# JacobYoung115/VisualSLAM

Measured on AMD Instinct MI355X. Metric: frames/sec @1080p (Harris + DoG keypoint detection), higher is better.
Workload: dtype u8

## Files before the change

### visualslam_amd/csrc/kernels_hdiff.hip.h

```cpp
#pragma once
#include <hip/hip_runtime.h>

#include <utility>
#include <vector>

#include "diff_taps.gen.h"
#include "kernels_strip.hip.h"
#include "vslam_internal.h"

namespace vslam {

typedef float hd_f2 __attribute__((ext_vector_type(2)));

template <class F, int... I>
__device__ __forceinline__ void hd_for_impl(F&& f, std::integer_sequence<int, I...>) {
    (f(std::integral_constant<int, I>{}), ...);
}
template <int N, class F>
__device__ __forceinline__ void hd_for(F&& f) {
    hd_for_impl(f, std::make_integer_sequence<int, N>{});
}

__host__ __device__ constexpr int hd_phys(int c) { return c + (c >> 4) * HD_PAD; }

template <class LV>
__host__ __device__ constexpr int hd_w(int k) { return k >= 0 && k < LV::n ? (int)LV::w[k] : 0; }

template <class LV>
__host__ __device__ constexpr int hd_coef(int e) {
    if (LV::form == 1) {
        for (int i = 0; i < LV::nd; ++i)
            if (LV::de[i] == e) return LV::dc[i];
        return 0;
    }
    return hd_w<LV>(e + LV::n / 2);
}

template <int O>
struct HdGeom {
    static constexpr int nmax = dtaps::Lvl<O, 5>::n;
    static constexpr int rmax = nmax / 2;
    static constexpr int HL = hd_left_halo(rmax);
    static_assert(dtaps::Lvl<O, 0>::n <= nmax && dtaps::Lvl<O, 4>::n <= nmax, "level 5 is the widest");
};

template <class LV, int HL>
__device__ __forceinline__ void hd_level(const hd_f2* __restrict__ lane, hd_f2 (&acc)[HD_J]) {
    constexpr int n = LV::n, r = n / 2;
    constexpr bool DIFF = LV::form == 1;
    constexpr int lo = DIFF ? -r - 1 : -r, hi = HD_J - 1 + r;
    constexpr int t0 = (HL + lo) & ~1, Q = (HL + hi - t0) / 2 + 1;
    hd_f2 seed = {0.f, 0.f};
    hd_for<HD_J>([&](auto j) { acc[decltype(j)::value] = hd_f2{0.f, 0.f}; });
    hd_for<Q>([&](auto q) {
        constexpr int t = t0 + 2 * decltype(q)::value;
        const float4 v = *reinterpret_cast<const float4*>(lane + hd_phys(t));
        const hd_f2 hv[2] = {hd_f2{v.x, v.y}, hd_f2{v.z, v.w}};
        hd_for<2>([&](auto b) {
            constexpr int x = t + decltype(b)::value - HL;
            if constexpr (DIFF) {
                constexpr int wk = hd_w<LV>(x + 1 + r);
                if constexpr (wk != 0) seed = __builtin_elementwise_fma(hd_f2((float)wk), hv[decltype(b)::value], seed);
            }
            hd_for<HD_J>([&](auto j) {
                constexpr int c = hd_coef<LV>(x - decltype(j)::value);
                if constexpr (c != 0)
                    acc[decltype(j)::value] = __builtin_elementwise_fma(hd_f2((float)c), hv[decltype(b)::value], acc[decltype(j)::value]);
            });
        });
    });
    if constexpr (DIFF) {
        acc[0] += seed;
        hd_for<HD_J - 1>([&](auto j) { acc[decltype(j)::value + 1] += acc[decltype(j)::value]; });
    }
}

template <int O>
__global__ __launch_bounds__(256) void k_gauss_h_diff(const uint16_t* __restrict__ h, size_t hframe, uint8_t* __restrict__ oct_out,
                                                       size_t pframe, int rows, int cols, int pitch, int npairs, int pw,
                                                       uint8_t* __restrict__ next_base, size_t nframe, int nrows, int ncols, int npitch) {
    using G = HdGeom<O>;
    extern __shared__ __attribute__((aligned(16))) uint32_t smem[];
    hd_f2* hp = reinterpret_cast<hd_f2*>(smem);
    const int tid = threadIdx.x;
    const int y0 = blockIdx.y * 2 * npairs;
    const size_t P = (size_t)rows * pitch;
    uint8_t* out = oct_out + blockIdx.z * pframe;
    const int ncs = (cols + HD_J - 1) / HD_J;
    const int ccount = G::HL + HD_J * ncs + G::rmax;
    const int n8 = cols >> 3, nb = ccount - 8 * n8;
    const bool active = tid < npairs * ncs;
    const int ip = tid / ncs, is = tid - ip * ncs;
    const hd_f2* lane = hp + ip * pw + is * (HD_J + HD_PAD);
    const int n8d = max(n8, 1);
    const int i_p0 = tid / n8d, i_k0 = tid - i_p0 * n8d, i_dp = 256 / n8d, i_dk = 256 - i_dp * n8d;
    const int b_p0 = tid / nb, b_i0 = tid - b_p0 * nb, b_dp = 256 / nb, b_di = 256 - b_dp * nb;
    uint32_t prev_e[2][4], prev_o[2][4];

    hd_for<VSLAM_NUM_LEVELS>([&](auto lc) {
        constexpr int L = decltype(lc)::value;
        const uint16_t* hl = h + blockIdx.z * hframe + (size_t)L * P;
        __syncthreads();
        for (int it = tid, p = i_p0, k = i_k0; it < npairs * n8; it += 256, p += i_dp, k += i_dk) {
            if (k >= n8) k -= n8, ++p;
            const uint4 a = *reinterpret_cast<const uint4*>(hl + (size_t)min(y0 + 2 * p, rows - 1) * pitch + 8 * k);
            const uint4 b = *reinterpret_cast<const uint4*>(hl + (size_t)min(y0 + 2 * p + 1, rows - 1) * pitch + 8 * k);
            float4* q = reinterpret_cast<float4*>(hp + p * pw + hd_phys(G::HL + 8 * k));
            const uint32_t av[4] = {a.x, a.y, a.z, a.w}, bv[4] = {b.x, b.y, b.z, b.w};
#pragma unroll
            for (int i = 0; i < 4; ++i)
                q[i] = make_float4((float)(av[i] & 0xffffu), (float)(bv[i] & 0xffffu), (float)(av[i] >> 16), (float)(bv[i] >> 16));
        }
        for (int it = tid, p = b_p0, i = b_i0; it < npairs * nb; it += 256, p += b_dp, i += b_di) {
            if (i >= nb) i -= nb, ++p;
            const int c = i < G::HL ? i : 8 * n8 + i;
            const int x = reflect101(c - G::HL, cols);
            const uint16_t* ra = hl + (size_t)min(y0 + 2 * p, rows - 1) * pitch;
            const uint16_t* rb = hl + (size_t)min(y0 + 2 * p + 1, rows - 1) * pitch;
            hp[p * pw + hd_phys(c)] = hd_f2{(float)ra[x], (float)rb[x]};
        }
        __syncthreads();
        if (active) {
            hd_f2 acc[HD_J];
            hd_level<dtaps::Lvl<O, L>, G::HL>(lane, acc);
            const int x = HD_J * is;
            hd_for<2>([&](auto rc) {
                constexpr int rho = decltype(rc)::value;
                const int y = y0 + 2 * ip + rho;
                uint32_t u[HD_J], g[4], d[4];
                hd_for<HD_J>([&](auto j) { u[decltype(j)::value] = (uint32_t)acc[decltype(j)::value][rho]; });
#pragma unroll
                for (int hw = 0; hw < 4; ++hw) {
                    const uint32_t e = __builtin_amdgcn_perm(u[4 * hw + 2], u[4 * hw + 0], 0x0c060c02);
                    const uint32_t o = __builtin_amdgcn_perm(u[4 * hw + 3], u[4 * hw + 1], 0x0c060c02);
                    g[hw] = __builtin_amdgcn_perm(o, e, 0x06020400);
                    if constexpr (L > 0)
                        d[hw] = __builtin_amdgcn_perm(pk_sub_sat_u16(o, prev_o[rho][hw]), pk_sub_sat_u16(e, prev_e[rho][hw]), 0x06020400);
                    prev_e[rho][hw] = e;
                    prev_o[rho][hw] = o;
                }
                if (y < rows) {
                    const size_t off = (size_t)y * pitch + x;
                    *reinterpret_cast<uint4*>(out + (size_t)L * P + off) = make_uint4(g[0], g[1], g[2], g[3]);
                    if constexpr (L > 0)
                        *reinterpret_cast<uint4*>(out + (size_t)(VSLAM_NUM_LEVELS + L - 1) * P + off) = make_uint4(d[0], d[1], d[2], d[3]);
                    if constexpr (L == 3 && rho == 0)
                        if (next_base && (y >> 1) < nrows && (x >> 1) < ncols)
                            *reinterpret_cast<uint2*>(next_base + blockIdx.z * nframe + (size_t)(y >> 1) * npitch + (x >> 1)) =
                                make_uint2(even_bytes(g[0], g[1]), even_bytes(g[2], g[3]));
                }
            });
        }
    });
}

template <int O, int L>
static bool hd_level_matches(const std::vector<uint16_t>& t) {
    using LV = dtaps::Lvl<O, L>;
    if ((int)t.size() != LV::n) return false;
    for (int k = 0; k < LV::n; ++k)
        if (t[k] != LV::w[k]) return false;
    std::vector<int> off, coef;
    if (diff_form(t.data(), LV::n, off, coef) != LV::form) return false;
    if (LV::form == 1) {
        if ((int)off.size() != LV::nd) return false;
        for (int i = 0; i < LV::nd; ++i)
            if (off[i] != LV::de[i] || coef[i] != LV::dc[i]) return false;
    }
    return true;
}
template <int O>
static bool hd_octave_matches(const std::vector<uint16_t> (&taps)[6]) {
    return hd_level_matches<O, 0>(taps[0]) && hd_level_matches<O, 1>(taps[1]) && hd_level_matches<O, 2>(taps[2]) &&
           hd_level_matches<O, 3>(taps[3]) && hd_level_matches<O, 4>(taps[4]) && hd_level_matches<O, 5>(taps[5]);
}

}
```

### visualslam_amd/csrc/vslam_hip.hip

```cpp
#include <hip/hip_runtime.h>

#include <algorithm>
#include <cstdio>
#include <cstdlib>
#include <cstring>
#include <deque>
#include <map>
#include <string>
#include <set>
#include <memory>
#include <vector>

#include "../../include/vslam.h"
#include "kernels_generic.hip.h"
#include "kernels_pyramid.hip.h"
#include "kernels_strip.hip.h"
#include "kernels_hdiff.hip.h"
#include "kernels_aux.hip.h"
#include "kernels_harris_strip.hip.h"
#include "kernels_orient.hip.h"
#include "kernels_orient_batch.hip.h"
#include "kernels_orient_pk.hip.h"
#include "kernels_compact.hip.h"
#include "kernels_sift.hip.h"
#include "kernels_extrema_dense.hip.h"
#include "vslam_batch_plan.h"
#include "vslam_internal.h"
#include "vslam_ctx.h"
#include "vslam_launch.h"
#include "vslam_mx.h"
#include "vslam_octave_launch.h"

using namespace vslam;


struct vslam_pyramid {
    vslam_ctx* ctx = nullptr;
    vslam_params params{};
    vslam_batch_layout layout{};
    vslam_pyramid_info info{};
    uint8_t* d_block = nullptr;
    uint8_t* d_bases = nullptr;
    size_t block_cap = 0, bases_cap = 0;
    size_t base_off[VSLAM_MAX_OCTAVES] = {};
};


static const char* const kKernelNames =
    "k_resize_linear2x\nk_blur_h_generic\nk_blur_v_generic\n"
    "k_dog5\nk_resize_nearest_half\nk_extrema\nk_pyr_octave\nk_pyr_octave_mx\n"
    "k_gauss_v_strip\nk_gauss_h_strip\nk_gauss_h_diff\nk_resize_linear2x_slide\nk_resize_nearest_half_v4\nk_extrema_w3\nk_extrema_dense\nk_localize_points\nk_orient_keypoints\nk_edge_response_windows\nk_level_gradients\nk_pack_rows\nk_edge_flags\nk_survivor_ranges\nk_orient_survivors\n"
    "k_extrema_pack\nk_harris_strip\nk_flag_count\nk_chunk_scan\nk_flag_scatter\nk_level_gradients\nk_sift_descriptors\nk_pack_offsets\nk_pack_copy\nk_count_totals\n"
    "k_desc_norms\nk_match_nn2\nk_match_merge\n"
    "k_guided_rows\nk_match_guided\nk_match_guided_merge\n"
    "k_guided_hf_rows\nk_guided_hf_kinds\nk_match_guided_hf\n"
    "k_match_nn2_mutual\nk_match_mutual_merge\nk_match_rnn_write\n"
    "k_epi_coords\nk_epi_models\nk_epi_score\nk_epi_select\nk_epi_flags\n"
    "k_refit_init\nk_refit_count\nk_refit_begin\nk_refit_dist\nk_refit_scale\nk_refit_moments\nk_refit_solve\n"
    "k_hom_models\nk_hom_score\nk_hom_select\nk_hom_flags\nk_hom_verdict\n"
    "k_pose_candidates\nk_pose_vote\nk_pose_select\nk_pose_points\n"
    "k_chain_link\nk_chain_ratio\nk_chain_median\nk_chain_walk\nk_chain_map\n"
    "k_res_corr\nk_res_gather\nk_res_models\nk_res_score\nk_res_select\nk_res_flags\n"
    "k_rr_init\nk_rr_pass\nk_rr_step\nk_rr_flags_zero\nk_rr_flags\n"
    "k_trk_next\nk_trk_walk\nk_trk_rows\n"
    "k_ba_init\nk_ba_points\nk_ba_cam_pass\nk_ba_cam_step\nk_ba_member_bits\nk_ba_points_final";


struct StreamSwap {
    vslam_ctx* c;
    hipStream_t saved;
    StreamSwap(vslam_ctx* ctx, hipStream_t s) : c(ctx), saved(ctx->stream) { c->stream = s; }
    ~StreamSwap() { c->stream = saved; }
};

static int raise_dyn_lds(vslam_ctx* c, const void* fn) {
    if (c->lds_raised.count(fn)) return VSLAM_OK;
    HIPCHK(c, hipFuncSetAttribute(fn, hipFuncAttributeMaxDynamicSharedMemorySize, kMaxDynLds));
    c->lds_raised.insert(fn);
    return VSLAM_OK;
}

static void* block_alloc(vslam_ctx* c, size_t bytes, size_t* cap) {
    int best = -1;
    for (int i = 0; i < (int)c->block_cache.size(); ++i) {
        const size_t sz = c->block_cache[i].first;
        if (sz >= bytes && sz <= 2 * bytes + (1 << 20) && (best < 0 || sz < c->block_cache[best].first)) best = i;
    }
    if (best >= 0) {
        void* p = c->block_cache[best].second;
        *cap = c->block_cache[best].first;
        c->block_cache.erase(c->block_cache.begin() + best);
        return p;
    }
    void* p = nullptr;
    if (hipMalloc(&p, bytes) != hipSuccess) {
        for (auto& b : c->block_cache) (void)hipFree(b.second);
        c->block_cache.clear();
        if (hipMalloc(&p, bytes) != hipSuccess) return nullptr;
    }
    *cap = bytes;
    return p;
}
static void block_release(vslam_ctx* c, void* p, size_t cap) {
    if (!p) return;
    if (c && c->block_cache.size() < 8 && cap <= ((size_t)1 << 30))
        c->block_cache.emplace_back(cap, p);
    else
        (void)hipFree(p);
}

int vslam::ws_reserve(vslam_ctx* c, size_t bytes) {
    if (bytes <= c->ws_cap) return VSLAM_OK;
    HIPCHK(c, hipStreamSynchronize(c->stream));
    for (int i = 0; i < vslam_ctx::kAux; ++i)
        if (c->aux[i]) HIPCHK(c, hipStreamSynchronize(c->aux[i]));
    if (c->ws) (void)hipFree(c->ws);
    c->ws = nullptr;
    c->ws_cap = 0;
    const size_t want = align_up(bytes + bytes / 8, 1 << 20);
    HIPCHK(c, hipMalloc((void**)&c->ws, want));
    c->ws_cap = want;
    return VSLAM_OK;
}

static bool stream_is_capturing(vslam_ctx* c) {
    hipStreamCaptureStatus cap = hipStreamCaptureStatusNone;
    if (hipStreamIsCapturing(c->stream, &cap) != hipSuccess) (void)hipGetLastError();
    return cap != hipStreamCaptureStatusNone;
}
#define NO_TABLE_IN_CAPTURE(ctx, what)                                                                                                      \
    if (stream_is_capturing(ctx))                                                                                                           \
    return fail(ctx, VSLAM_ERR_UNSUPPORTED, std::string(what) + ": its tap tables are not on the device yet and cannot be put there during a stream capture - " \
                                                                "run one warm-up call with the same parameters and the same matrix-path setting first")

enum TableKind { kTableBlur, kTableStrip, kTableTile, kTableMx, kTableOrient };

template <class T, class Fill>
static int get_table(vslam_ctx* c, TableKind kind, double v, int i, const char* what, size_t bytes, Fill fill, const T** out) {
    uint64_t vb;
    std::memcpy(&vb, &v, 8);
    const auto key = std::make_tuple((int)kind, vb, i);
    auto it = c->tables.find(key);
    if (it == c->tables.end()) {
        NO_TABLE_IN_CAPTURE(c, what);
        std::vector<char> host(bytes);
        TRY(fill(static_cast<void*>(host.data())));
        void* d = nullptr;
        HIPCHK(c, hipMalloc(&d, bytes));
        HIPCHK(c, hipMemcpy(d, host.data(), bytes, hipMemcpyHostToDevice));
        it = c->tables.emplace(key, d).first;
    }
    *out = static_cast<const T*>(it->second);
    return VSLAM_OK;
}

static inline void tap_pointers(const std::vector<uint16_t> taps[6], const uint16_t* tp[6]) {
    for (int l = 0; l < 6; ++l) tp[l] = taps[l].data();
}

static int get_taps(vslam_ctx* c, int n, double sigma, const uint16_t** out, int* n_eff) {
    std::vector<uint16_t> h;
    if (!gauss_taps_q8_trimmed(n, sigma, h)) return fail(c, VSLAM_ERR_INVALID, "invalid Gaussian kernel size");
    *n_eff = (int)h.size();
    return get_table(c, kTableBlur, sigma, n, "Gaussian blur", sizeof(uint16_t) * h.size(), [&](void* host) -> int {
        std::memcpy(host, h.data(), sizeof(uint16_t) * h.size());
        return VSLAM_OK;
    }, out);
}

static inline dim3 grid_rows(int cols, int rows, int frames = 1) { return dim3((cols + 255) / 256, rows, frames); }


namespace {
enum class OctPath { Tile0, Tile1, Strip, Generic };

struct OctPlan {
    OctPath path = OctPath::Generic;
    int ks[6] = {};
    double sg[6] = {};
    int ke[6] = {};
    std::vector<uint16_t> taps[6];
    int nmax = 0;
    int sh = 0;
    int hdiff = 0;
    int mx = 0;
};
}

static bool taps_fit_u8(const OctPlan& pl) {
    for (int l = 0; l < 6; ++l)
        for (uint16_t v : pl.taps[l])
            if (v > 255) return false;
    return true;
}

template <class CFG>
static bool matches_cfg(const int ks[6]) {
    for (int l = 0; l < 6; ++l)
        if (ks[l] != CFG::n(l)) return false;
    return true;
}

static OctPlan plan_octave(double sigma0, int o, int rows, int cols) {
    OctPlan pl;
    int& nmax = pl.nmax;
    for (int l = 0; l < 6; ++l) {
        pl.sg[l] = sigma_at(sigma0, o, l);
        pl.ks[l] = gauss_ksize_u8(pl.sg[l]);
        if (!gauss_taps_q8_trimmed(pl.ks[l], pl.sg[l], pl.taps[l])) return pl;
        pl.ke[l] = (int)pl.taps[l].size();
        nmax = std::max(nmax, pl.ke[l]);
    }
    if (!taps_fit_u8(pl)) return pl;
    if (matches_cfg<PyrCfgOct0>(pl.ke)) {
        pl.path = OctPath::Tile0;
    } else if (matches_cfg<PyrCfgOct1>(pl.ke)) {
        pl.path = OctPath::Tile1;
    } else if (nmax <= STRIP_MAXN) {
        pl.sh = strip_plan_sh(rows, cols, nmax);
        if (pl.sh) pl.path = OctPath::Strip;
        if (pl.path == OctPath::Strip && hdiff_fits(cols))
            pl.hdiff = hd_octave_matches<2>(pl.taps) ? 2 : hd_octave_matches<3>(pl.taps) ? 3 : 0;
    }
    if (pl.path != OctPath::Generic) pl.mx = mx_config_for(pl.ke);
    return pl;
}

static std::vector<OctPlan> plan_octaves(double sigma0, const vslam_batch_layout& L) {
    std::vector<OctPlan> plans;
    for (int o = 0; o < L.n_octaves; ++o) plans.push_back(plan_octave(sigma0, o, L.rows[o], L.cols[o]));
    return plans;
}

template <int SH, int RI>
static int launch_h_strip(vslam_ctx* c, const uint16_t* h, size_t hframe, const OctIO& io, const StripLaunch& sl, const StripTaps* taps) {
    TRY(raise_dyn_lds(c, reinterpret_cast<const void*>(&k_gauss_h_strip<SH, RI>)));
    LAUNCH_ON(c, "k_gauss_h_strip", c->launch_tag, c->stream, sl.h_lds, (k_gauss_h_strip<SH, RI>), dim3(1, sl.h_grid_y, io.nf), dim3(256), h,
              hframe, io.oct, io.pframe, io.rows, io.cols, io.pitch, sl.pw, taps, io.next_base, io.nframe, io.nrows, io.ncols, io.npitch);
    return VSLAM_OK;
}

template <int O>
static int launch_h_diff(vslam_ctx* c, const uint16_t* h, size_t hframe, const OctIO& io, const StripLaunch& sl) {
    TRY(raise_dyn_lds(c, reinterpret_cast<const void*>(&k_gauss_h_diff<O>)));
    TimedScope ts(c, "k_gauss_h_strip", c->launch_tag);
    LAUNCH_ON(c, "k_gauss_h_diff", c->launch_tag, c->stream, sl.h_lds, k_gauss_h_diff<O>, dim3(1, sl.h_grid_y, io.nf), dim3(256), h,
              hframe, io.oct, io.pframe, io.rows, io.cols, io.pitch, sl.npairs, sl.pw, io.next_base, io.nframe, io.nrows, io.ncols, io.npitch);
    return VSLAM_OK;
}

static int enqueue_strip_octave(vslam_ctx* c, double sigma0, int o, const OctPlan& pl, const OctIO& io, uint16_t* h) {
    const StripTaps* taps;
    TRY(get_table(c, kTableStrip, sigma0, o, "strip kernels", sizeof(StripTaps), [&](void* host) -> int {
        const uint16_t* tp[6];
        tap_pointers(pl.taps, tp);
        if (!strip_pack_taps(tp, pl.ke, *static_cast<StripTaps*>(host))) return fail(c, VSLAM_ERR_UNSUPPORTED, "strip kernels: taps out of range");
        return VSLAM_OK;
    }, &taps));
    const int rows = io.rows, cols = io.cols, nf = io.nf;
    static const bool hdiff_off = [] {
        const char* e = VSLAM_DIAG_ENV("VSLAM_HDIFF");
        return e && e[0] == '0';
    }();
    const int hd = hdiff_off ? 0 : pl.hdiff;
    const StripLaunch sl = hd == 2   ? strip_launch(rows, cols, nf, pl.sh, true, pl.nmax, HdGeom<2>::HL, HdGeom<2>::rmax)
                           : hd == 3 ? strip_launch(rows, cols, nf, pl.sh, true, pl.nmax, HdGeom<3>::HL, HdGeom<3>::rmax)
                                     : strip_launch(rows, cols, nf, pl.sh, false, pl.nmax);
    const StripVGeom vg = strip_v_geom(rows, pl.nmax);
    const size_t P = (size_t)rows * io.pitch;
    TRY(raise_dyn_lds(c, reinterpret_cast<const void*>(&k_gauss_v_strip)));
    LAUNCH_ON(c, "k_gauss_v_strip", o, c->stream, sl.v_lds, k_gauss_v_strip, dim3((cols + STRIP_W - 1) / STRIP_W, sl.lsplit, nf), dim3(256), io.base, io.bframe,
              h, 6 * P, rows, cols, io.pitch, vg.RM, vg.rhq, taps);
    c->launch_tag = o;
    if (sl.diff) return hd == 2 ? launch_h_diff<2>(c, h, 6 * P, io, sl) : launch_h_diff<3>(c, h, 6 * P, io, sl);
    switch (sl.SH * 8 + sl.RI) {
        case 16 * 8 + 4: return launch_h_strip<16, 4>(c, h, 6 * P, io, sl, taps);
        case 16 * 8 + 2: return launch_h_strip<16, 2>(c, h, 6 * P, io, sl, taps);
        case 16 * 8 + 1: return launch_h_strip<16, 1>(c, h, 6 * P, io, sl, taps);
        case 8 * 8 + 4: return launch_h_strip<8, 4>(c, h, 6 * P, io, sl, taps);
        case 4 * 8 + 4: return launch_h_strip<4, 4>(c, h, 6 * P, io, sl, taps);
        case 4 * 8 + 1: return launch_h_strip<4, 1>(c, h, 6 * P, io, sl, taps);
    }
    return fail(c, VSLAM_ERR_UNSUPPORTED, "strip kernels: no instantiation for the chosen strip shape");
}


static int enqueue_blur(vslam_ctx* c, const uint8_t* src, size_t sstep, size_t sframe, uint8_t* dst, size_t dstep,
                        size_t dframe, uint16_t* h, int rows, int cols, int nf, int n, double sigma) {
    const uint16_t* taps;
    int rc = get_taps(c, n, sigma, &taps, &n);
    if (rc) return rc;
    const size_t P = (size_t)rows * cols;
    LAUNCH(c, "k_blur_h_generic", k_blur_h_generic, grid_rows(cols, rows, nf), dim3(256), src, sstep, sframe, h, P,
           rows, cols, taps, n);
    LAUNCH(c, "k_blur_v_generic", k_blur_v_generic, grid_rows(cols, rows, nf), dim3(256), h, P, dst, dstep, dframe,
           rows, cols, taps, n);
    return VSLAM_OK;
}

template <class E>
static int enqueue_compaction(vslam_ctx* c, const E& ent, size_t entries, int nf, unsigned int* chunk_ws, unsigned int cap,
                              unsigned int* counts, int append) {
    const int nchunks = (int)((entries + CMP_CHUNK - 1) / CMP_CHUNK);
    if (nchunks == 0) {
        if (!append) HIPCHK(c, hipMemsetAsync(counts, 0, sizeof(unsigned int) * (size_t)nf, c->stream));
        return VSLAM_OK;
    }
    LAUNCH(c, "k_flag_count", k_flag_count<E>, dim3(nchunks, 1, nf), dim3(256), ent, chunk_ws, nchunks);
    LAUNCH(c, "k_chunk_scan", k_chunk_scan, dim3(nf), dim3(256), chunk_ws, nchunks, counts, append);
    LAUNCH(c, "k_flag_scatter", k_flag_scatter<E>, dim3(nchunks, 1, nf), dim3(256), ent, chunk_ws, nchunks, cap);
    return VSLAM_OK;
}
static inline size_t compaction_ws_elems(size_t entries, int nf) { return (size_t)nf * ((entries + CMP_CHUNK - 1) / CMP_CHUNK) + 64; }

size_t vslam::match_list_ws_elems(size_t fwords, int n_pairs) { return compaction_ws_elems(fwords, n_pairs); }
int vslam::enqueue_match_list(vslam_ctx* c, const unsigned long long* flags, size_t fwords, const vslam_nn2* nn, unsigned int qcap, int n_pairs,
                              unsigned int* chunk_ws, vslam_match* matches, unsigned int match_cap, unsigned int* match_counts) {
    const MatchEntries ent{flags, fwords, nn, qcap, matches};
    return enqueue_compaction(c, ent, fwords, n_pairs, chunk_ws, matches ? match_cap : 0u, match_counts, 0);
}

int vslam::enqueue_inlier_list(vslam_ctx* c, const unsigned long long* flags, size_t fwords, const vslam_match* matches, const unsigned int* match_counts,
                               unsigned int match_cap, int n_pairs, unsigned int* chunk_ws, vslam_match* inliers, unsigned int inlier_cap,
                               unsigned int* inlier_counts) {
    const EpipolarEntries ent{flags, fwords, matches, match_counts, match_cap, inliers};
    return enqueue_compaction(c, ent, fwords, n_pairs, chunk_ws, inliers ? inlier_cap : 0u, inlier_counts, 0);
}

static int ensure_loc_lut(vslam_ctx* c) {
    if (c->loc_lut) return VSLAM_OK;
    constexpr int n = LOC_LUT_N * LOC_LUT_N * LOC_LUT_N;
    float* lut = nullptr;
    HIPCHK(c, hipMalloc((void**)&lut, sizeof(float) * n));
    hipLaunchKernelGGL(k_build_localization_lut, dim3((n + 255) / 256), dim3(256), 0, c->stream, lut);
    const hipError_t e = hipGetLastError();
    if (e != hipSuccess) {
        (void)hipFree(lut);
        return fail(c, VSLAM_ERR_HIP, std::string("k_build_localization_lut: ") + hipGetErrorString(e));
    }
    c->loc_lut = lut;
    return VSLAM_OK;
}

static void fill_geom(const vslam_ctx* c, const vslam_params& p, const vslam_batch_layout& L, ExtGeom& g) {
    std::memset(&g, 0, sizeof(g));
    g.loc_lut = c->loc_lut;
    g.n_oct = L.n_octaves;
    g.window = p.extrema_window;
    g.pad = (p.extrema_window - 1) / 2;
    g.min_contrast = p.min_contrast;
    g.localize = p.localize;
    for (int o = 0; o < L.n_octaves; ++o) {
        g.rows[o] = L.rows[o];
        g.cols[o] = L.cols[o];
        g.pitch[o] = L.pitch[o];
        g.lat_rows[o] = L.lat_rows[o];
        g.lat_cols[o] = L.lat_cols[o];
        g.wpr[o] = L.lat_words[o];
        g.oct_off[o] = L.octave_offset[o];
        g.bits_off[o] = L.bits_offset[o];
    }
}

struct DogScratch {
    uint8_t* bases = nullptr;
    size_t bases_frame = 0;
    size_t base_off[VSLAM_MAX_OCTAVES] = {};
    uint16_t* h = nullptr;
    unsigned long long* lflags = nullptr;
    unsigned int* cws = nullptr;
    unsigned int* pbegin = nullptr;
    uint8_t* sitemap = nullptr;
    size_t site_frame = 0, site_off[VSLAM_MAX_OCTAVES] = {};
    int site_pitch[VSLAM_MAX_OCTAVES] = {};
    uint8_t* colmap = nullptr;
    size_t col_frame = 0, col_off[VSLAM_MAX_OCTAVES] = {};
};

static inline int site_pitch_of(int lat_cols) { return (lat_cols + 63) & ~63; }
static size_t col_octave_bytes(const vslam_batch_layout& L, int o) { return align_up((size_t)5 * mx_seams(L.cols[o]) * L.rows[o] * 2, 16); }

static size_t dog_h_elems(const vslam_batch_layout& L, const std::vector<OctPlan>& plans) {
    size_t m = 0;
    for (int o = 0; o < L.n_octaves; ++o) {
        const size_t P = (size_t)L.rows[o] * L.pitch[o];
        if (plans[o].path == OctPath::Strip) m = std::max(m, 6 * P);
        if (plans[o].path == OctPath::Generic) m = std::max(m, P);
    }
    return m;
}

static void dog_scratch_plan(WsPlan& ws, const vslam_batch_layout& L, const std::vector<OctPlan>& plans, int nf, DogScratch& s, bool sitemap = false) {
    if (sitemap) {
        size_t off = 0;
        for (int o = 0; o < L.n_octaves; ++o) {
            s.site_off[o] = off;
            s.site_pitch[o] = site_pitch_of(L.lat_cols[o]);
            off += (size_t)L.lat_rows[o] * s.site_pitch[o];
        }
        s.site_frame = off;
        ws.add(s.sitemap, (size_t)nf * off);
        size_t coff = 0;
        for (int o = 0; o < L.n_octaves; ++o) {
            s.col_off[o] = coff;
            coff += col_octave_bytes(L, o);
        }
        s.col_frame = coff;
        ws.add(s.colmap, (size_t)nf * coff + 16);
    }
    size_t sum_p = 0;
    for (int o = 0; o < L.n_octaves; ++o) {
        s.base_off[o] = sum_p;
        sum_p += (size_t)L.rows[o] * L.pitch[o];
    }
    s.bases_frame = sum_p;
    ws.add(s.bases, (size_t)nf * sum_p);
    ws.add(s.h, (size_t)nf * dog_h_elems(L, plans) + 128);
    ws.add(s.lflags, (size_t)nf * L.bits_frame_words);
    ws.add(s.cws, compaction_ws_elems(L.bits_frame_words, nf));
    ws.add(s.pbegin, nf);
}


template <class CFG>
static int enqueue_pyr_octave(vslam_ctx* c, double sigma0, int o, const OctPlan& pl, const OctIO& io) {
    const PyrTaps<CFG>* taps;
    TRY(get_table(c, kTableTile, sigma0, o, "octave kernel", sizeof(PyrTaps<CFG>), [&](void* host) -> int {
        const uint16_t* tp[6];
        tap_pointers(pl.taps, tp);
        pyr_pack_taps<CFG>(tp, *static_cast<PyrTaps<CFG>*>(host));
        return VSLAM_OK;
    }, &taps));
    TRY(raise_dyn_lds(c, reinterpret_cast<const void*>(&k_pyr_octave<CFG>)));
    const dim3 grid((io.cols + CFG::TW - 1) / CFG::TW, (io.rows + CFG::TH - 1) / CFG::TH, io.nf);
    LAUNCH_ON(c, "k_pyr_octave", o, c->stream, CFG::LDS_BYTES, k_pyr_octave<CFG>, grid, dim3(CFG::NT), io.base, io.bframe, io.oct, io.pframe, io.rows,
              io.cols, io.pitch, taps, io.next_base, io.nframe, io.nrows, io.ncols, io.npitch);
    return VSLAM_OK;
}

static int enqueue_pyr_octave_mx(vslam_ctx* c, double sigma0, int o, const OctPlan& pl, const OctIO& io, const MxScan* scan, int up2_step = 0) {
    const void* table;
    TRY(get_table(c, kTableMx, sigma0, o, "matrix-core octave kernel", mx_taps_bytes(pl.mx), [&](void* host) -> int {
        const uint16_t* tp[6];
        tap_pointers(pl.taps, tp);
        if (!mx_pack(pl.mx, tp, host)) return fail(c, VSLAM_ERR_UNSUPPORTED, "matrix-core octave kernel: a tap exceeds 127");
        HIPCHK(c, mx_prepare(pl.mx));
        return VSLAM_OK;
    }, &table));
    hipError_t e;
    {
        TimedScope ts(c, "k_pyr_octave_mx", o);
        e = mx_launch(pl.mx, c->stream, table, io, scan, up2_step);
    }
    HIPCHK(c, e);
    return VSLAM_OK;
}

static DenseGeom dense_geom(const vslam_batch_layout& L, int o, int min_contrast, int nf) {
    DenseGeom g;
    g.rows = L.rows[o], g.cols = L.cols[o], g.pitch = L.pitch[o];
    g.wpr = (g.cols + 63) / 64;
    g.min_contrast = min_contrast;
    g.P = (unsigned int)((size_t)g.rows * g.pitch);
    g.dog_off = (unsigned int)(L.octave_offset[o] + (size_t)VSLAM_NUM_LEVELS * g.P);
    const long waves_per_rowseg = 4L * (((g.cols + 3) / 4 + 255) / 256) * nf;
    const long segs_wanted = std::max<long>(1, 8192 / waves_per_rowseg);
    g.seg = (int)std::min<long>(XD_SEG_MAX, std::max<long>(4, (g.rows + segs_wanted - 1) / segs_wanted));
    return g;
}

namespace {
struct DogOut {
    uint8_t* pyr;
    size_t pframe;
    unsigned long long* bits = nullptr;
    bool do_extrema = false;
    vslam_point* points = nullptr;
    unsigned int* counts = nullptr;
};

static inline hipStream_t lane_stream(const vslam_ctx* c, Lane l) { return l == Lane::Main ? c->stream : c->aux[(int)l - 1]; }

static BatchPlanIn batch_plan_input(const vslam_ctx* c, const vslam_params& p, const vslam_batch_layout& L, const std::vector<OctPlan>& plans, size_t fstep) {
    BatchPlanIn in;
    in.n_octaves = L.n_octaves;
    for (int o = 0; o < L.n_octaves; ++o) {
        in.tiled[o] = plans[o].path == OctPath::Tile0 || plans[o].path == OctPath::Tile1;
        in.lattice[o] = L.lat_rows[o] > 0 && L.lat_cols[o] > 0;
        in.scan_ok[o] = mx_scan_supported(plans[o].mx);
    }
    in.up2_ok = L.n_octaves > 0 && L.rows[0] == 2 * p.rows && L.cols[0] == 2 * p.cols && fstep <= 0x7fffffff && mx_up2_supported(plans[0].mx);
    in.dog = L.n_octaves > 0;
    in.localize = p.localize, in.orient = p.orient, in.extrema_dense = p.extrema_dense, in.extrema_window = p.extrema_window;
    in.mx = c->mx;
    return in;
}

struct DogChunk {
    const vslam_params& p;
    const vslam_batch_layout& L;
    const std::vector<OctPlan>& plans;
    const uint8_t* frames;
    size_t fstep, fframe;
    int nf;
    DogScratch& s;
    DogOut out;
    BatchPlan plan;
    ExtGeom g{};
    MxScan scan[VSLAM_MAX_OCTAVES] = {};

    int begin(vslam_ctx* c) {
        const int nf_a = plan.nf_a;
        if (p.localize) TRY(ensure_loc_lut(c));
        fill_geom(c, p, L, g);
        if (!plan.up2_fused)
            LAUNCH(c, "k_resize_linear2x_slide", k_resize_linear2x_slide, dim3(((p.cols + 3) / 4 + 255) / 256, (p.rows + 15) / 16, nf_a), dim3(256),
                   frames, fstep, fframe, s.bases + s.base_off[0], s.bases_frame, L.pitch[0], p.rows, p.cols, 16);
        if (nf_a < nf) {
            const hipStream_t up = lane_stream(c, plan.up_lane);
            if (plan.up_waits_chunk) HIPCHK(c, hipStreamWaitEvent(up, c->ev_chunk, 0));
            StreamSwap sw(c, up);
            LAUNCH(c, "k_resize_linear2x_slide", k_resize_linear2x_slide, dim3(((p.cols + 3) / 4 + 255) / 256, (p.rows + 15) / 16, nf - nf_a), dim3(256),
                   frames + (size_t)nf_a * fframe, fstep, fframe, s.bases + s.base_off[0] + (size_t)nf_a * s.bases_frame, s.bases_frame, L.pitch[0],
                   p.rows, p.cols, 16);
// ... 1299 lines not shown
```

### visualslam_amd/csrc/vslam_octave_launch.h

```cpp
#pragma once
#include <algorithm>
#include <cstddef>
#include <initializer_list>

namespace vslam {

constexpr int STRIP_W = 64;
constexpr int HD_J = 16;
constexpr int HD_PAD = 2;
constexpr int kMaxDynLds = 150 * 1024;

struct StripVGeom {
    int RM, rhq;
    size_t lds;
};
constexpr StripVGeom strip_v_geom(int rows, int nmax) {
    const int RM = (nmax / 2 + 3) & ~3;
    const int rhq = (((rows + 3) & ~3) + 2 * RM + 16) / 4;
    return StripVGeom{RM, rhq, (size_t)rhq * STRIP_W * 4};
}

constexpr int strip_pw(int cols, int nmax) { return ((cols + 7) / 2 + nmax / 2 + 12 + 3) & ~3; }

constexpr int strip_item_capacity(int RI) { return RI == 4 ? 512 : 1024; }

constexpr int strip_sh(int cols) { return cols <= 1024 ? 16 : cols <= 2048 ? 8 : cols <= 4096 ? 4 : 0; }

constexpr int strip_plan_sh(int rows, int cols, int nmax) {
    const int sh = strip_sh(cols);
    return sh && strip_v_geom(rows, nmax).lds <= (size_t)kMaxDynLds && (size_t)sh * strip_pw(cols, nmax) * 4 <= (size_t)kMaxDynLds ? sh : 0;
}

constexpr int hd_left_halo(int rmax) { return (rmax + 2 + 15) & ~15; }
constexpr int hd_pw(int cols, int HL, int rmax) {
    const int ccount = HL + 16 * ((cols + HD_J - 1) / HD_J) + rmax;
    return (ccount + 1 + 15) / 16 * (16 + HD_PAD);
}
constexpr bool hdiff_fits(int cols) { return (cols + HD_J - 1) / HD_J <= 256; }

struct StripLaunch {
    int lsplit;
    size_t v_lds;
    bool diff;
    int npairs;
    int SH, RI;
    int h_grid_y;
    size_t h_lds;
    int pw;
};

inline StripLaunch strip_launch(int rows, int cols, int nf, int sh, bool hdiff, int nmax, int hd_HL = 0, int hd_rmax = 0) {
    StripLaunch s{};
    s.v_lds = strip_v_geom(rows, nmax).lds;
    const int strips = (cols + STRIP_W - 1) / STRIP_W;
    const int want = (256 + strips * nf - 1) / (strips * nf);
    s.lsplit = want >= 6 ? 6 : want >= 3 ? 3 : want >= 2 ? 2 : 1;
    if (hdiff) {
        const int ncs = (cols + HD_J - 1) / HD_J;
        s.pw = hd_pw(cols, hd_HL, hd_rmax);
        int npairs = std::max(1, std::min(8, 256 / ncs));
        while (npairs > 1 && ((size_t)npairs * s.pw * 8 > (size_t)kMaxDynLds || (long)((rows + 2 * npairs - 1) / (2 * npairs)) * nf < 256)) --npairs;
        s.diff = true;
        s.npairs = npairs;
        s.h_grid_y = (rows + 2 * npairs - 1) / (2 * npairs);
        s.h_lds = (size_t)npairs * s.pw * 8;
        return s;
    }
    s.pw = strip_pw(cols, nmax);
    while (sh > 4 && (long)((rows + sh - 1) / sh) * nf < 256) sh >>= 1;
    int ri = 4;
    if (sh == 4 && (long)((rows + 3) / 4) * nf < 256 && ((cols + 7) / 8) * 4 <= 512) {
        ri = 1;
    } else if (sh == 16) {
        const int ncg = (cols + 7) / 8;
        auto waste = [&](int r) {
            const long items = (long)ncg * (16 / r);
            if (items > strip_item_capacity(r)) return 1e9;
            return (double)((items + 63) / 64 * 64 - items) / (double)items;
        };
        for (int r : {2, 1})
            if (waste(r) + 0.02 < waste(ri)) ri = r;
    }
    s.SH = sh;
    s.RI = ri;
    s.h_grid_y = (rows + sh - 1) / sh;
    s.h_lds = (size_t)sh * s.pw * 4;
    return s;
}

constexpr bool pyr_tile_wide(int rows, int cols) {
    return (long)((cols + 255) / 256) * ((rows + 31) / 32) <= (long)((cols + 127) / 128) * ((rows + 63) / 64);
}

}
```

Before: 14890.

## Prefetch next level rows into registers and fill halo from LDS in hdiff kernel

```diff
diff --git a/visualslam_amd/csrc/kernels_hdiff.hip.h b/visualslam_amd/csrc/kernels_hdiff.hip.h
--- a/visualslam_amd/csrc/kernels_hdiff.hip.h
+++ b/visualslam_amd/csrc/kernels_hdiff.hip.h
@@ -87,39 +87,95 @@
     const size_t P = (size_t)rows * pitch;
     uint8_t* out = oct_out + blockIdx.z * pframe;
     const int ncs = (cols + HD_J - 1) / HD_J;
-    const int ccount = G::HL + HD_J * ncs + G::rmax;
-    const int n8 = cols >> 3, nb = ccount - 8 * n8;
+    const int n8 = cols >> 3, tl = cols & 7;
+    const int nh = hd_halo_cols(cols, G::HL, G::rmax);
     const bool active = tid < npairs * ncs;
     const int ip = tid / ncs, is = tid - ip * ncs;
     const hd_f2* lane = hp + ip * pw + is * (HD_J + HD_PAD);
-    const int n8d = max(n8, 1);
-    const int i_p0 = tid / n8d, i_k0 = tid - i_p0 * n8d, i_dp = 256 / n8d, i_dk = 256 - i_dp * n8d;
-    const int b_p0 = tid / nb, b_i0 = tid - b_p0 * nb, b_dp = 256 / nb, b_di = 256 - b_dp * nb;
+
+    constexpr int HT = hd_halo_trips(G::HL, G::rmax);
+    const uint16_t* h0 = h + blockIdx.z * hframe;
+    auto row_of = [&](int p, int rho) { return h0 + (size_t)min(y0 + 2 * p + rho, rows - 1) * pitch; };
+    const uint16_t *ia[2], *ib[2], *ta, *tb;
+    float4* iq[2];
+    hd_f2* tq;
+    bool iv[2];
+    {
+        const int n8d = max(n8, 1);
+        int p = tid / n8d, k = tid - p * n8d;
+        const int dp = 256 / n8d, dk = 256 - dp * n8d;
+        hd_for<2>([&](auto ic) {
+            constexpr int i = decltype(ic)::value;
+            if (k >= n8d) k -= n8d, ++p;
+            iv[i] = tid + 256 * i < npairs * n8;
+            const int pp = iv[i] ? p : 0, kk = iv[i] ? k : 0;
+            ia[i] = row_of(pp, 0) + 8 * kk;
+            ib[i] = row_of(pp, 1) + 8 * kk;
+            iq[i] = reinterpret_cast<float4*>(hp + pp * pw + hd_phys(G::HL + 8 * kk));
+            p += dp, k += dk;
+        });
+    }
+    const bool tv = tid < npairs * tl;
+    {
+        const int tld = max(tl, 1);
+        const int p = tv ? tid / tld : 0, x = tv ? 8 * n8 + tid - p * tld : 0;
+        ta = row_of(p, 0) + x;
+        tb = row_of(p, 1) + x;
+        tq = hp + p * pw + hd_phys(G::HL + x);
+    }
+    uint32_t hx[HT];
+    {
+        int p = tid / nh, i = tid - p * nh;
+        const int dp = 256 / nh, di = 256 - dp * nh;
+        hd_for<HT>([&](auto tc) {
+            constexpr int t = decltype(tc)::value;
+            if (i >= nh) i -= nh, ++p;
+            const int c = i < G::HL ? i : cols + i;
+            const int x = reflect101(c - G::HL, cols);
+            hx[t] = tid + 256 * t < npairs * nh ? (uint32_t)(p * pw + hd_phys(G::HL + x)) | (uint32_t)(p * pw + hd_phys(c)) << 16 : 0xffff0000u;
+            p += dp, i += di;
+        });
+    }
+
+    uint4 ra[2], rb[2];
+    uint16_t rta, rtb;
+    auto load_level = [&](auto lc) {
+        const size_t lo = (size_t)decltype(lc)::value * P;
+        hd_for<2>([&](auto ic) {
+            constexpr int i = decltype(ic)::value;
+            ra[i] = *reinterpret_cast<const uint4*>(ia[i] + lo);
+            rb[i] = *reinterpret_cast<const uint4*>(ib[i] + lo);
+        });
+        rta = ta[lo];
+        rtb = tb[lo];
+    };
     uint32_t prev_e[2][4], prev_o[2][4];
 
+    load_level(std::integral_constant<int, 0>{});
     hd_for<VSLAM_NUM_LEVELS>([&](auto lc) {
         constexpr int L = decltype(lc)::value;
-        const uint16_t* hl = h + blockIdx.z * hframe + (size_t)L * P;
+        if constexpr (L > 0) __syncthreads();
+        hd_for<2>([&](auto ic) {
+            constexpr int i = decltype(ic)::value;
+            if (iv[i]) {
+                const uint32_t av[4] = {ra[i].x, ra[i].y, ra[i].z, ra[i].w}, bv[4] = {rb[i].x, rb[i].y, rb[i].z, rb[i].w};
+#pragma unroll
+                for (int j = 0; j < 4; ++j)
+                    iq[i][j] = make_float4((float)(av[j] & 0xffffu), (float)(bv[j] & 0xffffu), (float)(av[j] >> 16), (float)(bv[j] >> 16));
+            }
+        });
+        if (tv) *tq = hd_f2{(float)rta, (float)rtb};
         __syncthreads();
-        for (int it = tid, p = i_p0, k = i_k0; it < npairs * n8; it += 256, p += i_dp, k += i_dk) {
-            if (k >= n8) k -= n8, ++p;
-            const uint4 a = *reinterpret_cast<const uint4*>(hl + (size_t)min(y0 + 2 * p, rows - 1) * pitch + 8 * k);
-            const uint4 b = *reinterpret_cast<const uint4*>(hl + (size_t)min(y0 + 2 * p + 1, rows - 1) * pitch + 8 * k);
-            float4* q = reinterpret_cast<float4*>(hp + p * pw + hd_phys(G::HL + 8 * k));
-            const uint32_t av[4] = {a.x, a.y, a.z, a.w}, bv[4] = {b.x, b.y, b.z, b.w};
-#pragma unroll
-            for (int i = 0; i < 4; ++i)
-                q[i] = make_float4((float)(av[i] & 0xffffu), (float)(bv[i] & 0xffffu), (float)(av[i] >> 16), (float)(bv[i] >> 16));
-        }
-        for (int it = tid, p = b_p0, i = b_i0; it < npairs * nb; it += 256, p += b_dp, i += b_di) {
-            if (i >= nb) i -= nb, ++p;
-            const int c = i < G::HL ? i : 8 * n8 + i;
-            const int x = reflect101(c - G::HL, cols);
-            const uint16_t* ra = hl + (size_t)min(y0 + 2 * p, rows - 1) * pitch;
-            const uint16_t* rb = hl + (size_t)min(y0 + 2 * p + 1, rows - 1) * pitch;
-            hp[p * pw + hd_phys(c)] = hd_f2{(float)ra[x], (float)rb[x]};
+        {
+            hd_f2 hv[HT];
+            hd_for<HT>([&](auto tc) { hv[decltype(tc)::value] = hp[hx[decltype(tc)::value] & 0xffffu]; });
+            hd_for<HT>([&](auto tc) {
+                constexpr int t = decltype(tc)::value;
+                if ((hx[t] >> 16) != 0xffffu) hp[hx[t] >> 16] = hv[t];
+            });
         }
         __syncthreads();
+        if constexpr (L + 1 < VSLAM_NUM_LEVELS) load_level(std::integral_constant<int, L + 1>{});
         if (active) {
             hd_f2 acc[HD_J];
             hd_level<dtaps::Lvl<O, L>, G::HL>(lane, acc);
diff --git a/visualslam_amd/csrc/vslam_hip.hip b/visualslam_amd/csrc/vslam_hip.hip
--- a/visualslam_amd/csrc/vslam_hip.hip
+++ b/visualslam_amd/csrc/vslam_hip.hip
@@ -219,7 +219,7 @@
     } else if (nmax <= STRIP_MAXN) {
         pl.sh = strip_plan_sh(rows, cols, nmax);
         if (pl.sh) pl.path = OctPath::Strip;
-        if (pl.path == OctPath::Strip && hdiff_fits(cols))
+        if (pl.path == OctPath::Strip && hdiff_fits(cols) && hdiff_stage_fits(cols))
             pl.hdiff = hd_octave_matches<2>(pl.taps) ? 2 : hd_octave_matches<3>(pl.taps) ? 3 : 0;
     }
     if (pl.path != OctPath::Generic) pl.mx = mx_config_for(pl.ke);
diff --git a/visualslam_amd/csrc/vslam_octave_launch.h b/visualslam_amd/csrc/vslam_octave_launch.h
--- a/visualslam_amd/csrc/vslam_octave_launch.h
+++ b/visualslam_amd/csrc/vslam_octave_launch.h
@@ -37,6 +37,10 @@
     return (ccount + 1 + 15) / 16 * (16 + HD_PAD);
 }
 constexpr bool hdiff_fits(int cols) { return (cols + HD_J - 1) / HD_J <= 256; }
+constexpr int hd_max_pairs(int cols) { return std::max(1, std::min(8, 256 / ((cols + HD_J - 1) / HD_J))); }
+constexpr int hd_halo_cols(int cols, int HL, int rmax) { return HL + HD_J * ((cols + HD_J - 1) / HD_J) - cols + rmax; }
+constexpr int hd_halo_trips(int HL, int rmax) { return (8 * (HL + HD_J - 1 + rmax) + 255) / 256; }
+constexpr bool hdiff_stage_fits(int cols) { return hd_max_pairs(cols) * (cols >> 3) <= 2 * 256 && hd_max_pairs(cols) * (cols & 7) <= 256; }
 
 struct StripLaunch {
     int lsplit;
@@ -56,9 +60,8 @@
     const int want = (256 + strips * nf - 1) / (strips * nf);
     s.lsplit = want >= 6 ? 6 : want >= 3 ? 3 : want >= 2 ? 2 : 1;
     if (hdiff) {
-        const int ncs = (cols + HD_J - 1) / HD_J;
         s.pw = hd_pw(cols, hd_HL, hd_rmax);
-        int npairs = std::max(1, std::min(8, 256 / ncs));
+        int npairs = hd_max_pairs(cols);
         while (npairs > 1 && ((size_t)npairs * s.pw * 8 > (size_t)kMaxDynLds || (long)((rows + 2 * npairs - 1) / (2 * npairs)) * nf < 256)) --npairs;
         s.diff = true;
         s.npairs = npairs;
```

Result: faster. 15170 (median of 6 runs) (+1.9%).
